# JuliaStats/Klara.jl

Hardware: AMD Instinct MI355X
Metric: MCMC transitions/sec (whole node), 100-dim Gaussian, 65k chains (higher is better)
Workload: dtype f64

## Files before the change

klara.jl_amd/csrc/klara_diagt.h:

```cpp
#pragma once
#include "klara_kernels.h"

#ifndef KLARA_DIAGT_Q
#define KLARA_DIAGT_Q 8
#endif
#define KLARA_DIAGT_CPW (64 / KLARA_DIAGT_Q)
#ifndef KLARA_DT_FENCE_EVERY
#define KLARA_DT_FENCE_EVERY 2
#endif
#ifndef KLARA_DT_SLICE_WF
#define KLARA_DT_SLICE_WF 4
#endif
#ifndef KLARA_DT_W1
#define KLARA_DT_W1 4
#endif
#ifndef KLARA_Q4_MALA_WF
#define KLARA_Q4_MALA_WF 3
#endif
#ifndef KLARA_DT_WF
#define KLARA_DT_WF 2
#endif
#ifdef KLARA_DT_PERSISTENT
#define KLARA_DT_GROUP_LOOP for (long long grp = kl.group0 + wave0; grp < kl.group_end && grp * CPW < p.nchains; grp += nwaves)
#else
#define KLARA_DT_GROUP_LOOP const long long grp = kl.group0 + wave0; if (grp < kl.group_end && grp * CPW < p.nchains)
#endif
#define KLARA_DT_PAIR_FENCE(pi) do { if (KLARA_DT_FENCE_EVERY > 0 && ((pi) + 1) % KLARA_DT_FENCE_EVERY == 0) __builtin_amdgcn_sched_barrier(0); } while (0)

struct KAuto {
    const int* cell_in;
    int* cell_out;
    unsigned long long* acc_ctr;
    int* mirror;
    unsigned long long thr_work;
    int my_mode;
    int fanout;
    int launch_idx;
};
#define KLARA_AUTO_NONE KAuto{ nullptr, nullptr, nullptr, nullptr, 0ull, 0, 1, 0 }

__device__ __forceinline__ unsigned wave_sum_u32(unsigned v)
{
#pragma unroll
    for (int m = 1; m < 64; m <<= 1) v += (unsigned)__builtin_amdgcn_ds_bpermute((int)((((unsigned)threadIdx.x & 63u) ^ (unsigned)m) << 2), (int)v);
    return v;
}
__shared__ unsigned klara_auto_wg[2];
__device__ __forceinline__ void auto_begin()
{
    if (threadIdx.x < 2) klara_auto_wg[threadIdx.x] = 0u;
}
__device__ __forceinline__ void auto_finish(const KAuto& ka, unsigned wave_acc)
{
    if (ka.acc_ctr == nullptr) return;
    const unsigned tot = wave_sum_u32(wave_acc);
    if ((threadIdx.x & 63) == 0) {
        atomicAdd(&klara_auto_wg[0], tot);
        if (atomicAdd(&klara_auto_wg[1], 1u) != (blockDim.x >> 6) - 1) return;
        const unsigned long long wg_tot = atomicAdd(&klara_auto_wg[0], 0u);
        const unsigned long long old = atomicAdd(ka.acc_ctr, (1ull << 40) | wg_tot);
        if ((old >> 40) == (unsigned long long)gridDim.x - 1) {
            const unsigned long long total = (old & ((1ull << 40) - 1)) + wg_tot;
            *ka.acc_ctr = 0ull;
            const int mode = (total << 16) > ka.thr_work ? 1 : 0;
            if (ka.cell_out != nullptr) for (int k = 0; k < ka.fanout; ++k) ka.cell_out[2 * k] = mode;
            if (ka.mirror != nullptr) {
                for (int k = 0; k < ka.fanout; ++k) {
                    __hip_atomic_store(ka.mirror + 4 * k + 1, (int)(total > 0x7fffffffull ? 0x7fffffffull : total), __ATOMIC_RELAXED, __HIP_MEMORY_SCOPE_SYSTEM);
                    __hip_atomic_store(ka.mirror + 4 * k, mode, __ATOMIC_RELAXED, __HIP_MEMORY_SCOPE_SYSTEM);
                    __hip_atomic_store(ka.mirror + 4 * k + 2, ka.launch_idx, __ATOMIC_RELEASE, __HIP_MEMORY_SCOPE_SYSTEM);
                }
            }
        }
    }
}

template <int NP, int Q>
struct PairCtx {
    int lane, q, cw;
    unsigned off0;
    bool last_ok;
    bool last_full;
};

template <int NP, int Q>
__device__ __forceinline__ PairCtx<NP, Q> make_pctx(int D)
{
    PairCtx<NP, Q> c;
    c.lane = threadIdx.x & 63;
    c.q = c.lane & (Q - 1);
    c.cw = c.lane / Q;
    c.off0 = (unsigned)((c.cw * D + 2 * c.q) * 8);
    c.last_ok = 2 * ((NP - 1) * Q + c.q) < D;
    c.last_full = 2 * ((NP - 1) * Q + c.q) + 1 < D;
    return c;
}
template <int NP, int Q>
__device__ __forceinline__ unsigned pair_off(const PairCtx<NP, Q>& c, int p)
{
    const unsigned o = c.off0 + (unsigned)(p * Q * 16);
    return (p == NP - 1 && !c.last_ok) ? KLARA_BUF_OOB : o;
}
template <int NP, int Q>
__device__ __forceinline__ void load_pairs(const PairCtx<NP, Q>& c, __amdgpu_buffer_rsrc_t w, double (&v)[2 * NP])
{
#pragma unroll
    for (int p = 0; p < NP; ++p) {
        const kd_uint4 t = __builtin_amdgcn_raw_buffer_load_b128(w, pair_off<NP, Q>(c, p), 0, 0);
        v[2 * p] = __builtin_bit_cast(double, kd_uint2{ t.x, t.y });
        v[2 * p + 1] = __builtin_bit_cast(double, kd_uint2{ t.z, t.w });
        if (p == NP - 1 && !c.last_full) v[2 * p + 1] = 0.0;
    }
}
template <int NP, int Q>
__device__ __forceinline__ void store_pairs(const PairCtx<NP, Q>& c, __amdgpu_buffer_rsrc_t w, const double (&v)[2 * NP])
{
#pragma unroll
    for (int p = 0; p < NP; ++p) {
        const kd_uint2 a = __builtin_bit_cast(kd_uint2, v[2 * p]), b = __builtin_bit_cast(kd_uint2, v[2 * p + 1]);
        if (p < NP - 1) {
            __builtin_amdgcn_raw_buffer_store_b128(kd_uint4{ a.x, a.y, b.x, b.y }, w, pair_off<NP, Q>(c, p), 0, 0);
        } else {
            const unsigned o = pair_off<NP, Q>(c, p);
            __builtin_amdgcn_raw_buffer_store_b64(a, w, o, 0, 0);
            __builtin_amdgcn_raw_buffer_store_b64(b, w, c.last_full ? o + 8u : KLARA_BUF_OOB, 0, 0);
        }
    }
}
template <int NP, int Q>
__device__ __forceinline__ void load_pairs_if(const PairCtx<NP, Q>& c, __amdgpu_buffer_rsrc_t w, bool on, double (&v)[2 * NP])
{
#pragma unroll
    for (int p = 0; p < NP; ++p) {
        const kd_uint4 t = __builtin_amdgcn_raw_buffer_load_b128(w, on ? pair_off<NP, Q>(c, p) : KLARA_BUF_OOB, 0, 0);
        v[2 * p] = __builtin_bit_cast(double, kd_uint2{ t.x, t.y });
        v[2 * p + 1] = __builtin_bit_cast(double, kd_uint2{ t.z, t.w });
        if (p == NP - 1 && !c.last_full) v[2 * p + 1] = 0.0;
    }
}
template <int NP, int Q>
__device__ __forceinline__ void store_pairs_if(const PairCtx<NP, Q>& c, __amdgpu_buffer_rsrc_t w, bool on, const double (&v)[2 * NP])
{
#pragma unroll
    for (int p = 0; p < NP; ++p) {
        const kd_uint2 a = __builtin_bit_cast(kd_uint2, v[2 * p]), b = __builtin_bit_cast(kd_uint2, v[2 * p + 1]);
        const unsigned o = on ? pair_off<NP, Q>(c, p) : KLARA_BUF_OOB;
        if (p < NP - 1) {
            __builtin_amdgcn_raw_buffer_store_b128(kd_uint4{ a.x, a.y, b.x, b.y }, w, o, 0, 0);
        } else {
            __builtin_amdgcn_raw_buffer_store_b64(a, w, o, 0, 0);
            __builtin_amdgcn_raw_buffer_store_b64(b, w, (on && c.last_full) ? o + 8u : KLARA_BUF_OOB, 0, 0);
        }
    }
}
template <int NP, int Q>
__device__ __forceinline__ void diagt_fold(const PairCtx<NP, Q>& c, __amdgpu_buffer_rsrc_t wsum, __amdgpu_buffer_rsrc_t wsq, bool fold,
                                        bool& loaded, long long& held, const double (&x)[2 * NP], double (&sm)[2 * NP], double (&sq)[2 * NP])
{
    const bool need = fold && !loaded;
    if (__any(need)) {
        double ts[2 * NP], tq[2 * NP];
        load_pairs_if<NP, Q>(c, wsum, need, ts);
        load_pairs_if<NP, Q>(c, wsq, need, tq);
#pragma unroll
        for (int e = 0; e < 2 * NP; ++e) { sm[e] = need ? ts[e] : sm[e]; sq[e] = need ? tq[e] : sq[e]; }
        loaded = loaded || need;
    }
    const double hf = fold ? (double)held : 0.0;
#pragma unroll
    for (int e = 0; e < 2 * NP; ++e) {
        const double a = sm[e] + hf * x[e], b = sq[e] + hf * (x[e] * x[e]);
        sm[e] = fold ? a : sm[e]; sq[e] = fold ? b : sq[e];
    }
    held = fold ? 0 : held;
}

#ifndef KLARA_DT_RMW_CHUNK
#define KLARA_DT_RMW_CHUNK 3
#endif
template <int NP, int Q>
__device__ __forceinline__ void diagt_fold_atomic(const PairCtx<NP, Q>& c, gdouble* sum0, gdouble* sq0, bool fold, long long& held, const double (&x)[2 * NP])
{
    typedef __attribute__((address_space(1))) double* gptr;
    if (fold) {
        const double hf = (double)held;
        const gptr ps = (gptr)((__attribute__((address_space(1))) char*)sum0 + c.off0), pq = (gptr)((__attribute__((address_space(1))) char*)sq0 + c.off0);
#pragma unroll
        for (int p = 0; p < NP; ++p) {
            const bool ok0 = p < NP - 1 || c.last_ok, ok1 = p < NP - 1 || c.last_full;
            if (ok0) {
                (void)__builtin_amdgcn_global_atomic_fadd_f64(ps + p * Q * 2, hf * x[2 * p]);
                (void)__builtin_amdgcn_global_atomic_fadd_f64(pq + p * Q * 2, hf * (x[2 * p] * x[2 * p]));
            }
            if (ok1) {
                (void)__builtin_amdgcn_global_atomic_fadd_f64(ps + p * Q * 2 + 1, hf * x[2 * p + 1]);
                (void)__builtin_amdgcn_global_atomic_fadd_f64(pq + p * Q * 2 + 1, hf * (x[2 * p + 1] * x[2 * p + 1]));
            }
        }
    }
    held = fold ? 0 : held;
}
template <int NP, int Q>
__device__ __forceinline__ void diagt_fold_rmw(const PairCtx<NP, Q>& c, __amdgpu_buffer_rsrc_t wsum, __amdgpu_buffer_rsrc_t wsq, bool fold,
                                               long long& held, const double (&x)[2 * NP])
{
    const double hf = fold ? (double)held : 0.0;
    constexpr int CH = KLARA_DT_RMW_CHUNK;
#pragma unroll
    for (int p0 = 0; p0 < NP; p0 += CH) {
        kd_uint4 ts[CH], tq[CH];
#pragma unroll
        for (int k = 0; k < CH; ++k) {
            if (p0 + k < NP) {
                const unsigned o = fold ? pair_off<NP, Q>(c, p0 + k) : KLARA_BUF_OOB;
                ts[k] = __builtin_amdgcn_raw_buffer_load_b128(wsum, o, 0, 0);
                tq[k] = __builtin_amdgcn_raw_buffer_load_b128(wsq, o, 0, 0);
            }
        }
#pragma unroll
        for (int k = 0; k < CH; ++k) {
            if (p0 + k < NP) {
                const int p = p0 + k;
                const unsigned o = fold ? pair_off<NP, Q>(c, p) : KLARA_BUF_OOB;
                const double s0 = __builtin_bit_cast(double, kd_uint2{ ts[k].x, ts[k].y }) + hf * x[2 * p];
                const double s1 = __builtin_bit_cast(double, kd_uint2{ ts[k].z, ts[k].w }) + hf * x[2 * p + 1];
                const double q0 = __builtin_bit_cast(double, kd_uint2{ tq[k].x, tq[k].y }) + hf * (x[2 * p] * x[2 * p]);
                const double q1 = __builtin_bit_cast(double, kd_uint2{ tq[k].z, tq[k].w }) + hf * (x[2 * p + 1] * x[2 * p + 1]);
                const kd_uint2 a = __builtin_bit_cast(kd_uint2, s0), b = __builtin_bit_cast(kd_uint2, s1);
                const kd_uint2 e = __builtin_bit_cast(kd_uint2, q0), f = __builtin_bit_cast(kd_uint2, q1);
                if (p < NP - 1) {
                    __builtin_amdgcn_raw_buffer_store_b128(kd_uint4{ a.x, a.y, b.x, b.y }, wsum, o, 0, 0);
                    __builtin_amdgcn_raw_buffer_store_b128(kd_uint4{ e.x, e.y, f.x, f.y }, wsq, o, 0, 0);
                } else {
                    const unsigned o1 = (fold && c.last_full) ? o + 8u : KLARA_BUF_OOB;
                    __builtin_amdgcn_raw_buffer_store_b64(a, wsum, o, 0, 0); __builtin_amdgcn_raw_buffer_store_b64(b, wsum, o1, 0, 0);
                    __builtin_amdgcn_raw_buffer_store_b64(e, wsq, o, 0, 0); __builtin_amdgcn_raw_buffer_store_b64(f, wsq, o1, 0, 0);
                }
            }
        }
    }
    held = fold ? 0 : held;
}

template <int NP, int Q>
__device__ __forceinline__ void load_pair_param(const PairCtx<NP, Q>& c, const gdouble* base, int D, double dflt, double (&v)[2 * NP])
{
#pragma unroll
    for (int p = 0; p < NP; ++p) {
        const int i = 2 * (p * Q + c.q);
        v[2 * p] = dflt; v[2 * p + 1] = dflt;
        if (base != nullptr && i < D) v[2 * p] = base[i];
        if (base != nullptr && i + 1 < D) v[2 * p + 1] = base[i + 1];
    }
}

template <int Q> struct PairShare {
    static constexpr int STEP = Q <= 8 ? 8 / Q : 0;
    static constexpr bool second(int p) { return STEP != 0 && ((p / (STEP ? STEP : 1)) & 1) != 0; }
};
template <int NP, int Q>
__device__ __forceinline__ void pair_words(const PairCtx<NP, Q>& c, unsigned long long seed, unsigned long long gchain,
                                           unsigned long long t, int p, uint32_t (&stash)[4], uint32_t& wa, uint32_t& wb)
{
    constexpr int STEP = PairShare<Q>::STEP, S1 = STEP ? STEP : 1;
    if (PairShare<Q>::second(p)) {
        wa = stash[2 * (p % S1)]; wb = stash[2 * (p % S1) + 1];
    } else {
        const uint32_t idx = (uint32_t)(p * Q + c.q);
        const bool pad = p == NP - 1 && !c.last_ok;
        const kd_u32x4 b = kd_stream_block(seed, gchain, t, pad ? idx : kd_pair_block(idx));
        if constexpr (STEP != 0) {
            wa = b.x; wb = b.y;
            stash[2 * (p % S1)] = b.z; stash[2 * (p % S1) + 1] = b.w;
        } else {
            const bool hb = !pad && kd_pair_half(idx) != 0u;
            wa = hb ? b.z : b.x; wb = hb ? b.w : b.y;
        }
    }
}
template <int NP, int Q, bool SCTAB = false>
__device__ __forceinline__ void pair_normals(const PairCtx<NP, Q>& c, unsigned long long seed, unsigned long long gchain,
                                             unsigned long long t, int p, uint32_t (&stash)[4], double& z0, double& z1, double& u1, double& lg1)
{
    uint32_t wa, wb;
    pair_words<NP, Q>(c, seed, gchain, t, p, stash, wa, wb);
    kd_normal_pair_w_t<SCTAB>(wa, wb, &z0, &z1, &u1, &lg1);
    KLARA_PIN(z0); KLARA_PIN(z1);
    if (p == NP - 1 && !c.last_ok) z0 = 0.0;
    if (p == NP - 1 && !c.last_full) z1 = 0.0;
}
template <int NP, int Q>
__device__ __forceinline__ void pair_issue(const PairCtx<NP, Q>& c, unsigned long long seed, unsigned long long gchain,
                                           unsigned long long t, int p, uint32_t (&stash)[4], kd_pair_reads& rd)
{
    uint32_t wa, wb;
    pair_words<NP, Q>(c, seed, gchain, t, p, stash, wa, wb);
    kd_normal_pair_issue(wa, wb, &rd);
    __builtin_amdgcn_sched_barrier(0);
}
template <int NP, int Q>
__device__ __forceinline__ void pair_finish(const PairCtx<NP, Q>& c, int p, const kd_pair_reads& rd, double& z0, double& z1, double& u1, double& lg1)
{
    kd_normal_pair_finish(&rd, &z0, &z1, &u1, &lg1);
    KLARA_PIN(z0); KLARA_PIN(z1);
    if (p == NP - 1 && !c.last_ok) z0 = 0.0;
    if (p == NP - 1 && !c.last_full) z1 = 0.0;
}

template <int V> struct kd_int { static constexpr int value = V; };
template <int FROM, int TO, class F>
__device__ __forceinline__ void kd_static_for(F&& f)
{
    if constexpr (FROM < TO) { f(kd_int<FROM>{}); kd_static_for<FROM + 1, TO>(f); }
}

template <bool UNITW>
__device__ __forceinline__ void diag_elem(double x, double w, double m2w, double m, double& term, double& grad)
{
    const double dd = UNITW ? x : x - m;
    term = UNITW ? dd * dd : w * (dd * dd);
    grad = UNITW ? -2.0 * dd : m2w * dd;
}

template <int SAMPLER, int NP, int Q, bool ONESTEP, bool TUNE>
__host__ __device__ constexpr int diagt_min_waves()
{
    return NP <= 8 ? (ONESTEP && SAMPLER != KLARA_SAMPLER_HMC ? KLARA_DT_W1 : KLARA_DT_WF)
                   : (Q == 4 && NP <= 13 && !TUNE ? (SAMPLER == KLARA_SAMPLER_MALA ? KLARA_Q4_MALA_WF : 2) : 1);
}

#ifndef KLARA_SCTAB_MIN_STEPS
#define KLARA_SCTAB_MIN_STEPS 8
#endif
template <int SAMPLER, int NP, int Q, bool ONESTEP, bool UNITW, bool MON, bool TUNE>
__host__ __device__ constexpr bool diagt_sctab()
{
    return SAMPLER == KLARA_SAMPLER_MALA && ((Q == 4 && NP == 13) || (Q == 8 && NP == 7)) && !ONESTEP && UNITW && MON && !TUNE;
}
#ifndef KLARA_Q4_SCTAB_WG
#define KLARA_Q4_SCTAB_WG 256
#endif
template <int Q, bool SCTAB>
__host__ __device__ constexpr int diagt_wg_threads() { return SCTAB && Q == 4 ? KLARA_Q4_SCTAB_WG : 256; }

#ifdef KLARA_USER_PAIR_TARGET
#define KLARA_PAIR_CALL(a, b, P, g0, g1) klara_user_pair((a), (b), (P), D, (const double*)p.cdata, (long long)p.cndata, (g0), (g1))
#else
#define KLARA_PAIR_CALL(a, b, P, g0, g1) 0.0
#endif
template <int SAMPLER, int NP, int Q, bool ONESTEP, bool UNITW, bool MON, bool TUNE = false, bool DA = false, bool USERPAIR = false, bool SCTAB = false>
__global__ __launch_bounds__((diagt_wg_threads<Q, SCTAB>()), (SAMPLER == KLARA_SAMPLER_SLICE && NP <= 8 && !MON && !TUNE ? KLARA_DT_SLICE_WF : diagt_min_waves<SAMPLER, NP, Q, ONESTEP, TUNE>()))
void k_diagt(const KParams* __restrict__ pp, const KLaunch kl, const KAuto ka)
{
#ifndef KLARA_USER_PAIR_TARGET
    static_assert(!USERPAIR, "pair closures exist in run-time compiled translation units only");
#endif
    static_assert(!USERPAIR || (UNITW && Q >= 8), "pair closures: 8 or more lanes per chain");
    static_assert(!SCTAB || (!ONESTEP && !USERPAIR && SAMPLER != KLARA_SAMPLER_SLICE), "the remainder table: fused launches of the built-in MH / MALA / HMC kernels");
    if (ka.cell_in != nullptr && *ka.cell_in != ka.my_mode) return;
    static_assert(!(ONESTEP && (MON || TUNE)), "monitored / tuned jobs run the committing kernel");
    static_assert(!DA || (TUNE && SAMPLER == KLARA_SAMPLER_HMC), "dual averaging: tuned HMC");
    constexpr bool PLAIN = !TUNE;
    constexpr int E = 2 * NP, CPW = 64 / Q;
    constexpr bool NEEDG = SAMPLER == KLARA_SAMPLER_MALA || SAMPLER == KLARA_SAMPLER_HMC;
    constexpr bool SLICE = SAMPLER == KLARA_SAMPLER_SLICE;
    static_assert(!(SLICE && ONESTEP), "the slice sampler moves every chain: it runs the committing kernel");
    constexpr bool MEMSUM = MON && !TUNE && Q == 4 && (SAMPLER == KLARA_SAMPLER_MH || SAMPLER == KLARA_SAMPLER_MALA);
    const KParams& p = *pp;
    __shared__ __attribute__((aligned(16))) double lds_w[UNITW ? 2 : 2 * NP * Q];
    __shared__ __attribute__((aligned(16))) double lds_mu[UNITW ? 2 : 2 * NP * Q];
    __shared__ __attribute__((aligned(16))) double lds_m2w[UNITW ? 2 : 2 * NP * Q];
    if (!UNITW) {
        for (int i = (int)threadIdx.x; i < 2 * NP * Q; i += (int)blockDim.x) {
            lds_w[i] = (p.gw != nullptr && i < p.D) ? p.gw[i] : 1.0;
            lds_mu[i] = (p.gmu != nullptr && i < p.D) ? p.gmu[i] : 0.0;
            lds_m2w[i] = -2.0 * lds_w[i];
        }
    }
    auto_begin();
    if constexpr (SCTAB) kd_sincos_rem_to_lds();
    kd_tables_to_lds();
    if (p.clock_probe != nullptr && blockIdx.x == (gridDim.x >> 1) && threadIdx.x == 0) {
        p.clock_probe[2] = __builtin_amdgcn_s_memtime(); p.clock_probe[3] = __builtin_amdgcn_s_memrealtime();
    }
    const int D = p.D;
    const PairCtx<NP, Q> cx = make_pctx<NP, Q>(D);
    const int nsteps = ONESTEP ? 1 : kl.nsteps;
    guchar* const accept_out = p.accept != nullptr ? p.accept + kl.t0 * (unsigned long long)p.nchains : nullptr;

    double sig[E];
    const auto wv = [&](int e) { return UNITW ? 1.0 : lds_w[2 * ((e >> 1) * Q + cx.q) + (e & 1)]; };
    const auto mv = [&](int e) { return UNITW ? 0.0 : lds_mu[2 * ((e >> 1) * Q + cx.q) + (e & 1)]; };
    const auto m2wv = [&](int e) { return UNITW ? -2.0 : lds_m2w[2 * ((e >> 1) * Q + cx.q) + (e & 1)]; };
    const auto wvl = [&](int e) { return UNITW ? 1.0 : *(volatile const double*)&lds_w[2 * ((e >> 1) * Q + cx.q) + (e & 1)]; };
    const auto mvl = [&](int e) { return UNITW ? 0.0 : *(volatile const double*)&lds_mu[2 * ((e >> 1) * Q + cx.q) + (e & 1)]; };
    const auto m2wvl = [&](int e) { return UNITW ? -2.0 : *(volatile const double*)&lds_m2w[2 * ((e >> 1) * Q + cx.q) + (e & 1)]; };
    if (SAMPLER == KLARA_SAMPLER_MH) load_pair_param<NP, Q>(cx, p.vecparam, D, 1.0, sig);
    const double gconst = USERPAIR ? 0.0 : p.gconst;

    const int acc_slot = (D + 1) >> 1;
    const bool acc_free = acc_slot < NP * Q && !PairShare<Q>::second(NP - 1);
    const int acc_lane = (cx.lane - cx.q) + (acc_slot & (Q - 1));

    const long long nwaves = (long long)gridDim.x * (blockDim.x >> 6);
    const long long wave0 = __builtin_amdgcn_readfirstlane((int)(blockIdx.x * (blockDim.x >> 6) + (threadIdx.x >> 6)));
    unsigned wave_acc = 0;
    KLARA_DT_GROUP_LOOP {
        const long long first_chain = grp * CPW;
        const long long left = p.nchains - first_chain;
        const int here = left < CPW ? (int)left : CPW;
        const bool chain_ok = cx.cw < here;
        const long long chain = first_chain + cx.cw;
        const unsigned long long gchain = (unsigned long long)(p.chain_offset + chain);
        const __amdgpu_buffer_rsrc_t wx = group_window(p.X, first_chain, here, D);
        const __amdgpu_buffer_rsrc_t wg = group_window(p.GR, first_chain, here, D);

        double x[E];
        load_pairs<NP, Q>(cx, wx, x);
        const auto user_pair = [&](int pi, double a, double b, double& nt, double& g0, double& g1) {
            double u0 = 0.0, u1 = 0.0, u = 0.0;
            const bool ok0 = pi < NP - 1 || cx.last_ok, ok1 = pi < NP - 1 || cx.last_full;
            if (ok0) u = KLARA_PAIR_CALL(a, b, pi * Q + cx.q, &u0, &u1);
            nt = ok0 ? -u : 0.0; g0 = ok0 ? u0 : 0.0; g1 = ok1 ? u1 : 0.0;
        };
        const auto grad_of = [&](const double (&v)[E], double (&out)[E]) {
            if constexpr (USERPAIR) {
#pragma unroll
                for (int pi = 0; pi < NP; ++pi) { double nt; user_pair(pi, v[2 * pi], v[2 * pi + 1], nt, out[2 * pi], out[2 * pi + 1]); }
            } else {
#pragma unroll
                for (int e = 0; e < E; ++e) { double term_; diag_elem<UNITW>(v[e], wv(e), m2wv(e), mv(e), term_, out[e]); }
            }
        };
        double lt = p.LT[chain_ok ? chain : 0];
        unsigned long long nacc = 0;
        bool stuck = false;
        const bool do_sum = MON && p.sum != nullptr;
        double sm[MEMSUM ? 2 : E], sq[MEMSUM ? 2 : E];
        bool sums_loaded = false;
        long long held = 0;
        __amdgpu_buffer_rsrc_t wsum = wx, wsq = wx;
        if (do_sum) {
#pragma unroll
            for (int e = 0; e < (MEMSUM ? 2 : E); ++e) { sm[e] = 0.0; sq[e] = 0.0; }
            wsum = group_window(p.sum, first_chain, here, D); wsq = group_window(p.sumsq, first_chain, here, D);
            held = p.held[chain_ok ? chain : 0];
        }
        int sphase = kl.save_phase0;
        long long scol = kl.save_col0;
        const bool per_chain_tune = KCNT && !KPOOLED;
        const long long c0 = chain_ok ? chain : 0;
        TuneRegs tn;
        if (per_chain_tune) tn = { p.tune_step[c0], p.tune_accepted[c0], p.tune_proposed[c0], p.tune_totproposed[c0], 0, 0.0, 0.0 };
        else if (KPOOLED) tn = { p.tune_step[0], p.tune_accepted[0], 0, 0, 0, 0.0, 0.0 };
        else tn = { DA ? p.tune_step[c0] : p.step0, 0, 0, 0, 0, 0.0, 0.0 };
        if (DA) { tn.epsbar = p.da_epsbar[c0]; tn.hbar = p.da_hbar[c0]; }
        const long long acc0 = tn.accepted;
        tn.phase = per_chain_tune ? (int)(tn.proposed % p.period) : 0;

        struct { unsigned long long seed; long long burnin, nsteps_total, hist_cols, held_inc; int thinning; double sqrt_step0, inv_step0; } lc = {};
        if constexpr (SCTAB) {
            lc.seed = p.seed; lc.burnin = p.burnin; lc.nsteps_total = p.nsteps_total; lc.hist_cols = p.hist_cols; lc.thinning = (int)p.thinning;
            lc.held_inc = __builtin_amdgcn_readfirstlane(do_sum ? 1 : 0); lc.sqrt_step0 = p.sqrt_step0; lc.inv_step0 = p.inv_step0;
            KLARA_PIN_S(lc.seed); KLARA_PIN_S(lc.burnin); KLARA_PIN_S(lc.nsteps_total); KLARA_PIN_S(lc.hist_cols); KLARA_PIN_S(lc.thinning);
            KLARA_PIN_S(lc.held_inc); KLARA_PIN_S(lc.sqrt_step0); KLARA_PIN_S(lc.inv_step0);
        }
#define KLARA_LC(f) (SCTAB ? lc.f : p.f)
        for (int s = 0; s < nsteps; ++s) {
            const unsigned long long t = kl.t0 + (unsigned long long)s;
            if (KCNT) tune_count_proposal(p, tn);
            double xp[E];
            const auto put_xp = [&](int pi, double a, double b) { xp[2 * pi] = a; xp[2 * pi + 1] = b; };
            constexpr int NR = Q == 4 ? 2 : 1;
            double red[3 * NR] = {}, red1[1], red2[2];
            double u_last = 0.5, lg_last = 0.0;
            uint32_t nstash[4] = { 0u, 0u, 0u, 0u };
            bool acc;
            double ltp, a_da = 0.0;

            constexpr bool ZFIRST = (ONESTEP || Q != 4) && SAMPLER != KLARA_SAMPLER_HMC && !SLICE;
            double z[ZFIRST ? E : 2];
            kd_pair_reads rd[2];
            if (ZFIRST) {
                if constexpr (SCTAB) pair_issue<NP, Q>(cx, KLARA_LC(seed), gchain, t, 0, nstash, rd[0]);
#pragma unroll
                for (int pi = 0; pi < NP; ++pi) {
                    if constexpr (SCTAB) {
                        if (pi + 1 < NP) pair_issue<NP, Q>(cx, KLARA_LC(seed), gchain, t, pi + 1, nstash, rd[(pi + 1) & 1]);
                        pair_finish<NP, Q>(cx, pi, rd[pi & 1], z[2 * pi], z[2 * pi + 1], u_last, lg_last);
                        __builtin_amdgcn_sched_barrier(0);
                    } else {
                        pair_normals<NP, Q, SCTAB>(cx, KLARA_LC(seed), gchain, t, pi, nstash, z[2 * pi], z[2 * pi + 1], u_last, lg_last);
                        KLARA_DT_PAIR_FENCE(pi);
                    }
                }
            }
            if constexpr (SLICE) {
                if (do_sum && __any(held > 0))
                    diagt_fold<NP, Q>(cx, wsum, wsq, held > 0, sums_loaded, held, x, sm, sq);
            }
            if (SLICE) {
                acc = true;
                const __amdgpu_buffer_rsrc_t wwid = __builtin_amdgcn_make_buffer_rsrc((void*)p.vecparam, 0, D * 8, 0x00020000);
#pragma unroll
                for (int e = 0; e < E; ++e) {
                    const int i = 2 * ((e >> 1) * Q + cx.q) + (e & 1);
                    const bool live = chain_ok && i < D;
                    const uint32_t base = (uint32_t)(live ? i : 0) << KLARA_SLICE_ATT_BITS;
                    const kd_u32x4 b0 = kd_stream_block(KLARA_LC(seed), gchain, t, base);
                    const double lgu = kd_log_u01(kd_uniform_xy(b0));
                    const double ru = kd_uniform_zw(b0);
                    const double wi_t = UNITW ? 1.0 : wv(e), mi_t = UNITW ? 0.0 : mv(e);
                    const double xi = x[e], wd = __builtin_bit_cast(double, __builtin_amdgcn_raw_buffer_load_b64(wwid, (unsigned)(live ? i : 0) * 8u, 0, 0));
                    double tcur, gd_;
                    if constexpr (USERPAIR) { double g1_; user_pair(e >> 1, x[e & ~1], x[e | 1], tcur, gd_, g1_); }
                    else diag_elem<UNITW>(xi, wi_t, -2.0 * wi_t, mi_t, tcur, gd_);
                    double Li = xi - ru * wd;
                    double Ri = xi + (1.0 - ru) * wd;
                    const auto term_of = [&](double cand) -> double {
                        double tc, gd;
                        if constexpr (USERPAIR) { double g1; user_pair(e >> 1, (e & 1) ? x[e & ~1] : cand, (e & 1) ? cand : x[e | 1], tc, gd, g1); }
                        else diag_elem<UNITW>(cand, wi_t, -2.0 * wi_t, mi_t, tc, gd);
                        return tc;
                    };
                    if (p.stepout) {
                        double dl = tcur - term_of(Li);
                        int guard = 0;
                        while (true) {
                            bool go = live && !stuck && (dl > lgu);
                            if (go && ++guard > KLARA_SLICE_MAX_ATT) { stuck = true; go = false; }
                            if (!__any(go)) break;
                            const double Ln = Li - wd;
                            const double dn = tcur - term_of(go ? Ln : Li);
                            if (go) { Li = Ln; dl = dn; }
                        }
                        double dr = tcur - term_of(Ri);
                        guard = 0;
                        while (true) {
                            bool go = live && !stuck && (dr > lgu);
                            if (go && ++guard > KLARA_SLICE_MAX_ATT) { stuck = true; go = false; }
                            if (!__any(go)) break;
                            const double Rn = Ri + wd;
                            const double dn = tcur - term_of(go ? Rn : Ri);
                            if (go) { Ri = Rn; dr = dn; }
                        }
                    }
                    double xprime = xi;
                    bool done = !live || stuck;
                    kd_u32x4 ab = b0;
                    for (uint32_t a = 1;; ++a) {
                        if (!done && a > KLARA_SLICE_MAX_ATT) { stuck = true; done = true; }
                        if (!__any(!done)) break;
                        if (a & 1u) ab = kd_stream_block(KLARA_LC(seed), gchain, t, kd_slice_attempt_slot(base, a));
                        const double u = (a & 1u) ? kd_uniform_xy(ab) : kd_uniform_zw(ab);
                        const double cand = u * (Ri - Li) + Li;
                        const double tc = term_of(done ? xprime : cand);
                        if (!done) {
                            xprime = cand;
                            if (tcur - tc > lgu) done = true;
                            else if (cand > xi) Ri = cand;
                            else if (cand < xi) Li = cand;
                            else { stuck = true; done = true; }
                        }
                    }
                    if (live && !stuck) x[e] = xprime;
                }
                red1[0] = 0.0;
                if constexpr (USERPAIR) {
#pragma unroll
                    for (int pi = 0; pi < NP; ++pi) { double nt, g0_, g1_; user_pair(pi, x[2 * pi], x[2 * pi + 1], nt, g0_, g1_); red1[0] = red1[0] + nt; }
                } else {
#pragma unroll
                for (int e = 0; e < E; ++e) { double te, gd; diag_elem<UNITW>(x[e], wv(e), m2wv(e), mv(e), te, gd); red1[0] = red1[0] + te; }
                }
                group_allreduce<1>(red1, Q, cx.lane);
                lt = gconst - red1[0];
                ltp = lt;
#pragma unroll
                for (int e = 0; e < E; ++e) xp[e] = x[e];
            } else if (SAMPLER == KLARA_SAMPLER_MH) {
                const auto mh_elem = [&](int e, double ze, int r) -> double {
                    const double xe = x[e] + sig[e] * ze;
                    double term, gd;
                    diag_elem<UNITW>(xe, wv(e), m2wv(e), mv(e), term, gd);
                    red[r] = red[r] + term;
                    return xe;
                };
#pragma unroll
                for (int pi = 0; pi < NP; ++pi) {
                    double z0 = ZFIRST ? z[(2 * pi) % (ZFIRST ? E : 2)] : 0.0, z1 = ZFIRST ? z[(2 * pi + 1) % (ZFIRST ? E : 2)] : 0.0;
                    if (!ZFIRST) pair_normals<NP, Q, SCTAB>(cx, KLARA_LC(seed), gchain, t, pi, nstash, z0, z1, u_last, lg_last);
                    const int r = (NR == 2 && (pi & 1)) ? 3 : 0;
                    if constexpr (USERPAIR) {
                        const double a = x[2 * pi] + sig[2 * pi] * z0, b = x[2 * pi + 1] + sig[2 * pi + 1] * z1;
                        double nt, g0, g1;
                        user_pair(pi, a, b, nt, g0, g1);
                        red[r] = red[r] + nt;
                        put_xp(pi, a, b);
                    } else {
                        const double a = mh_elem(2 * pi, z0, r), b = mh_elem(2 * pi + 1, z1, r);
                        put_xp(pi, a, b);
                    }
                    if (!ZFIRST) KLARA_DT_PAIR_FENCE(pi);
                }
                if (NR == 2) {
                    red2[0] = red[0]; red2[1] = red[3];
                    group_allreduce<2>(red2, Q, cx.lane);
                    red1[0] = red2[0] + red2[1];
                } else {
                    red1[0] = red[0];
                    group_allreduce<1>(red1, Q, cx.lane);
                }
                ltp = gconst - red1[0];
                const double ratio = ltp - lt;
                acc = ratio > 0.0;
                if (acc_free) acc = acc || ratio > lane_bcast(lg_last, acc_lane);
                else if (!acc && ratio > KD_LOG_UMIN_GUARD)
                    acc = ratio > kd_log_u01(kd_accept_uniform(kd_stream_block(KLARA_LC(seed), gchain, t, (uint32_t)acc_slot)));
            } else if (SAMPLER == KLARA_SAMPLER_MALA) {
                const double h_ = tn.step, halfh = 0.5 * h_, sq = KCNT ? __builtin_sqrt(h_) : KLARA_LC(sqrt_step0);
                const double half_inv_h = 0.5 * (KCNT ? 1.0 / h_ : KLARA_LC(inv_step0));
                const double neg_h = -h_;
                constexpr bool FROM_TERM = UNITW && PLAIN;
                const auto mala_elem = [&](int e, double ze, int r, bool first) -> double {
                    double term, ge = 0.0, gpe;
                    if constexpr (!UNITW) diag_elem<UNITW>(x[e], wv(e), m2wv(e), mv(e), term, ge);
                    const double m_ = UNITW ? x[e] + neg_h * x[e] : x[e] + halfh * ge;
                    const double xe = m_ + sq * ze;
                    diag_elem<UNITW>(xe, wv(e), m2wv(e), mv(e), term, gpe);
                    red[r] = first ? term : red[r] + term;
                    const double q1 = m_ - xe;
                    red[r + 1] = first ? (q1 * q1) * half_inv_h : red[r + 1] + (q1 * q1) * half_inv_h;
                    const double mup = UNITW ? xe + neg_h * xe : xe + halfh * gpe;
                    const double q2 = mup - x[e];
                    red[r + 2] = first ? (q2 * q2) * half_inv_h : red[r + 2] + (q2 * q2) * half_inv_h;
                    return xe;
                };
#pragma unroll
                for (int pi = 0; pi < NP; ++pi) {
                    double z0 = ZFIRST ? z[(2 * pi) % (ZFIRST ? E : 2)] : 0.0, z1 = ZFIRST ? z[(2 * pi + 1) % (ZFIRST ? E : 2)] : 0.0;
                    if constexpr (!ZFIRST && SCTAB) {
                        if (pi == 0) pair_issue<NP, Q>(cx, KLARA_LC(seed), gchain, t, 0, nstash, rd[0]);
                        pair_finish<NP, Q>(cx, pi, rd[pi & 1], z0, z1, u_last, lg_last);
                        if (pi + 1 < NP) pair_issue<NP, Q>(cx, KLARA_LC(seed), gchain, t, pi + 1, nstash, rd[(pi + 1) & 1]);
                    } else if (!ZFIRST) pair_normals<NP, Q, SCTAB>(cx, KLARA_LC(seed), gchain, t, pi, nstash, z0, z1, u_last, lg_last);
                    const int r = (NR == 2 && (pi & 1)) ? 3 : 0;
                    if constexpr (USERPAIR) {
                        double nt, ge0, ge1, gp0, gp1;
                        user_pair(pi, x[2 * pi], x[2 * pi + 1], nt, ge0, ge1);
                        const double m0 = x[2 * pi] + halfh * ge0, m1 = x[2 * pi + 1] + halfh * ge1;
                        const double a = m0 + sq * z0, b = m1 + sq * z1;
                        user_pair(pi, a, b, nt, gp0, gp1);
                        red[r] = red[r] + nt;
                        const double q10 = m0 - a, q11 = m1 - b;
                        red[r + 1] = red[r + 1] + (q10 * q10) * half_inv_h;
                        red[r + 1] = red[r + 1] + (q11 * q11) * half_inv_h;
                        const double q20 = (a + halfh * gp0) - x[2 * pi], q21 = (b + halfh * gp1) - x[2 * pi + 1];
                        red[r + 2] = red[r + 2] + (q20 * q20) * half_inv_h;
                        red[r + 2] = red[r + 2] + (q21 * q21) * half_inv_h;
                        put_xp(pi, a, b);
                    } else {
                        const double a = mala_elem(2 * pi, z0, r, FROM_TERM && pi < NR), b = mala_elem(2 * pi + 1, z1, r, false);
                        put_xp(pi, a, b);
                    }
                    if constexpr (!ZFIRST && SCTAB) __builtin_amdgcn_sched_barrier(0);
                    else if (!ZFIRST) KLARA_DT_PAIR_FENCE(pi);
                }
                group_allreduce<3 * NR>(red, Q, cx.lane);
                if (NR == 2) { red[0] = red[0] + red[3]; red[1] = red[1] + red[4]; red[2] = red[2] + red[5]; }
                ltp = gconst - red[0];
                double ratio = ltp - lt;
                ratio += red[1];
                ratio -= red[2];
                acc = ratio > 0.0;
                if (acc_free) acc = acc || ratio > lane_bcast(lg_last, acc_lane);
                else if (!acc && ratio > KD_LOG_UMIN_GUARD)
                    acc = ratio > kd_log_u01(kd_accept_uniform(kd_stream_block(KLARA_LC(seed), gchain, t, (uint32_t)acc_slot)));
            } else {
                const double eps = tn.step, halfe = 0.5 * eps;
                double mom[E], gp[E];
                double k0[NR] = {};
#pragma unroll
                for (int pi = 0; pi < NP; ++pi) {
                    pair_normals<NP, Q, SCTAB>(cx, KLARA_LC(seed), gchain, t, pi, nstash, mom[2 * pi], mom[2 * pi + 1], u_last, lg_last);
                    const int r = (NR == 2 && (pi & 1)) ? 1 : 0;
                    k0[r] = k0[r] + mom[2 * pi] * mom[2 * pi];
                    k0[r] = k0[r] + mom[2 * pi + 1] * mom[2 * pi + 1];
                }
                group_allreduce<NR>(k0, Q, cx.lane);
                if (NR == 2) k0[0] = k0[0] + k0[1];
                const double H0 = lt - 0.5 * k0[0];
#pragma unroll
                for (int e = 0; e < E; ++e) xp[e] = x[e];
                constexpr bool KFOLD = UNITW && !USERPAIR;
                if constexpr (!KFOLD) grad_of(x, gp);
                const int nl = DA ? (chain_ok ? da_nleaps(p, eps) : 1) : p.nleaps;
#pragma unroll
                for (int e = 0; e < E; ++e) {
                    if constexpr (KFOLD) mom[e] = kd_fma(-eps, x[e], mom[e]);
                    else mom[e] = kd_fma(halfe, gp[e], mom[e]);
                }
                const int nlmax = DA ? wave_max_int(nl) : nl;
                for (int l = 0; l < nlmax; ++l) {
                    const bool go = !DA || l < nl;
                    const double kf = l + 1 < nl ? eps : halfe;
                    const double nkf2 = -2.0 * kf;
                    if constexpr (USERPAIR) {
#pragma unroll
                        for (int pi = 0; pi < NP; ++pi) {
                            const double xa = kd_fma(eps, mom[2 * pi], xp[2 * pi]), xb = kd_fma(eps, mom[2 * pi + 1], xp[2 * pi + 1]);
                            xp[2 * pi] = go ? xa : xp[2 * pi]; xp[2 * pi + 1] = go ? xb : xp[2 * pi + 1];
                            double nt, ga, gb;
                            user_pair(pi, xp[2 * pi], xp[2 * pi + 1], nt, ga, gb);
                            gp[2 * pi] = go ? ga : gp[2 * pi]; gp[2 * pi + 1] = go ? gb : gp[2 * pi + 1];
                            const double na = kd_fma(kf, gp[2 * pi], mom[2 * pi]), nb = kd_fma(kf, gp[2 * pi + 1], mom[2 * pi + 1]);
                            mom[2 * pi] = go ? na : mom[2 * pi]; mom[2 * pi + 1] = go ? nb : mom[2 * pi + 1];
                        }
                    } else {
#pragma unroll
                        for (int e = 0; e < E; ++e) {
                            const double x1 = kd_fma(eps, mom[e], xp[e]);
                            xp[e] = go ? x1 : xp[e];
                            if constexpr (KFOLD) {
                                const double m2 = kd_fma(nkf2, xp[e], mom[e]);
                                mom[e] = go ? m2 : mom[e];
                            } else {
                                double term, g1;
                                diag_elem<UNITW>(xp[e], 1.0, m2wvl(e), mvl(e), term, g1);
                                gp[e] = go ? g1 : gp[e];
                                const double m2 = kd_fma(kf, gp[e], mom[e]);
                                mom[e] = go ? m2 : mom[e];
                            }
                        }
                    }
                }
                if constexpr (USERPAIR) {
#pragma unroll
                    for (int pi = 0; pi < NP; ++pi) {
                        double nt, ga, gb;
                        user_pair(pi, xp[2 * pi], xp[2 * pi + 1], nt, ga, gb);
                        red[0] = red[0] + nt;
                        red[1] = red[1] + mom[2 * pi] * mom[2 * pi];
                        red[1] = red[1] + mom[2 * pi + 1] * mom[2 * pi + 1];
                    }
                } else {
#pragma unroll
                for (int e = 0; e < E; ++e) {
                    double term, gd;
                    diag_elem<UNITW>(xp[e], wv(e), m2wv(e), mv(e), term, gd);
                    const int r = (NR == 2 && ((e >> 1) & 1)) ? 3 : 0;
                    red[r] = red[r] + term;
                    red[r + 1] = red[r + 1] + mom[e] * mom[e];
                }
                }
                if (NR == 2) {
                    double red4[4] = { red[0], red[1], red[3], red[4] };
                    group_allreduce<4>(red4, Q, cx.lane);
                    red2[0] = red4[0] + red4[2]; red2[1] = red4[1] + red4[3];
                } else {
                    red2[0] = red[0]; red2[1] = red[1];
                    group_allreduce<2>(red2, Q, cx.lane);
                }
                ltp = gconst - red2[0];
                const double H1 = ltp - 0.5 * red2[1];
                const double ratio = H1 - H0;
                const double ex = kd_exp(ratio);
                const double a = 1.0 < ex ? 1.0 : ex;
                a_da = a;
                const double u = acc_free ? lane_bcast(u_last, acc_lane)
                                          : kd_accept_uniform(kd_stream_block(KLARA_LC(seed), gchain, t, (uint32_t)acc_slot));
                acc = u < a;
            }

            if (accept_out != nullptr && chain_ok && cx.q == 0) accept_out[(long long)s * p.nchains + chain] = acc ? 1 : 0;
            if (KCNT && acc && !SLICE) tn.accepted += 1;
            if (DA) da_update(p, tn, (long long)t + 1, a_da);
            if (per_chain_tune && !DA) tuning_block(p, tn);
            else if (DA && per_chain_tune && tn.phase == 0 && (long long)t + 1 <= p.da_nadapt) {
                tn.totproposed += tn.proposed; tn.accepted = 0; tn.proposed = 0;
            }
            if constexpr (ONESTEP) {
                wave_acc += (acc && chain_ok && cx.q == 0) ? 1u : 0u;
                if (acc) {
                    store_pairs<NP, Q>(cx, wx, xp);
                    if (NEEDG) { double gq[E]; grad_of(xp, gq); store_pairs<NP, Q>(cx, wg, gq); }
                    if (chain_ok && cx.q == 0) { p.LT[chain] = ltp; p.naccept[chain] += 1ull; }
                }
            } else {
                nacc += acc ? 1ull : 0ull;
                if (!SLICE && do_sum && __any(chain_ok && acc && held > 0)) {
                    const bool fold = chain_ok && acc && held > 0;
#ifdef KLARA_DT_FOLD_RMW
                    if constexpr (MEMSUM) diagt_fold_rmw<NP, Q>(cx, wsum, wsq, fold, held, x);
#else
                    if constexpr (MEMSUM) diagt_fold_atomic<NP, Q>(cx, p.sum + first_chain * D, p.sumsq + first_chain * D, fold, held, x);
#endif
                    else diagt_fold<NP, Q>(cx, wsum, wsq, fold, sums_loaded, held, x, sm, sq);
                }
                if (acc) {
#pragma unroll
                    for (int e = 0; e < E; ++e) x[e] = xp[e];
                    lt = ltp;
                }
            }
            const long long i1 = (long long)t + 1;
            if (MON && i1 > KLARA_LC(burnin) && i1 <= KLARA_LC(nsteps_total)) {
                if (sphase == 0) {
                    if constexpr (SCTAB) held += lc.held_inc;
                    else if (do_sum) held += 1;
                    if (scol < KLARA_LC(hist_cols)) {
                        const long long col0 = scol * p.nchains + first_chain;
                        if (p.hist != nullptr) store_pairs<NP, Q>(cx, group_window(p.hist, col0, here, D), x);
                        if (NEEDG && p.hist_g != nullptr) { double gq[E]; grad_of(x, gq); store_pairs<NP, Q>(cx, group_window(p.hist_g, col0, here, D), gq); }
                        if (p.hist_lt != nullptr && chain_ok && cx.q == 0) p.hist_lt[scol * p.nchains + chain] = lt;
                    }
                    ++scol;
                }
                sphase = (sphase + 1 == (SCTAB ? lc.thinning : (int)p.thinning)) ? 0 : sphase + 1;
            }
        }
        if (do_sum) {
            if constexpr (!MEMSUM) {
                if (__any(sums_loaded)) {
                    store_pairs_if<NP, Q>(cx, wsum, sums_loaded, sm);
                    store_pairs_if<NP, Q>(cx, wsq, sums_loaded, sq);
                }
            }
            if (chain_ok && cx.q == 0) p.held[chain] = held;
        }
        if (SLICE && stuck && chain_ok) klara_raise(p.error_flag, KLARA_ERR_SLICE_STUCK);
        if (!ONESTEP) wave_acc += (chain_ok && cx.q == 0) ? (unsigned)nacc : 0u;
        if (!ONESTEP && nacc != 0) {
            store_pairs<NP, Q>(cx, wx, x);
            if (NEEDG) { double gq[E]; grad_of(x, gq); store_pairs<NP, Q>(cx, wg, gq); }
            if (chain_ok && cx.q == 0) { p.LT[chain] = lt; p.naccept[chain] += nacc; }
        }
        if (TUNE && chain_ok && cx.q == 0) {
            if (DA) { p.tune_step[chain] = tn.step; p.da_epsbar[chain] = tn.epsbar; p.da_hbar[chain] = tn.hbar; }
            if (per_chain_tune) {
                p.tune_step[chain] = tn.step; p.tune_accepted[chain] = tn.accepted;
                p.tune_proposed[chain] = tn.proposed; p.tune_totproposed[chain] = tn.totproposed;
            } else if (KPOOLED && KCNT) {
                atomicAdd((unsigned long long*)p.pooled_accepted, (unsigned long long)(tn.accepted - acc0));
            }
        }
    }
    if (p.clock_probe != nullptr && blockIdx.x == (gridDim.x >> 1) && threadIdx.x == 0) {
        p.clock_probe[0] = __builtin_amdgcn_s_memtime(); p.clock_probe[1] = __builtin_amdgcn_s_memrealtime();
    }
    auto_finish(ka, wave_acc);
#undef KLARA_LC
}

template <int NP, int Q, bool USERPAIR = false>
__global__ __launch_bounds__(256) void k_diagt_init(const KParams p, int needgrad)
{
#ifndef KLARA_USER_PAIR_TARGET
    static_assert(!USERPAIR, "pair closures exist in run-time compiled translation units only");
#endif
    constexpr int E = 2 * NP, CPW = 64 / Q;
    const int D = p.D;
    const PairCtx<NP, Q> cx = make_pctx<NP, Q>(D);
    const long long grp = __builtin_amdgcn_readfirstlane((int)(blockIdx.x * (blockDim.x >> 6) + (threadIdx.x >> 6)));
    const long long first_chain = grp * CPW;
    const long long left = p.nchains - first_chain;
    const int here = left < CPW ? (left > 0 ? (int)left : 0) : CPW;
    const bool chain_ok = cx.cw < here;
    const long long chain = first_chain + cx.cw;
    double w[E], mu[E], x[E], g[E], red[1] = { 0.0 };
    load_pair_param<NP, Q>(cx, p.gw, D, 1.0, w);
    load_pair_param<NP, Q>(cx, p.gmu, D, 0.0, mu);
    load_pairs<NP, Q>(cx, group_window(p.X, first_chain, here, D), x);
    bool bad = false;
    if constexpr (USERPAIR) {
#pragma unroll
        for (int pi = 0; pi < NP; ++pi) {
            double u0 = 0.0, u1 = 0.0, u = 0.0;
            const bool ok0 = pi < NP - 1 || cx.last_ok, ok1 = pi < NP - 1 || cx.last_full;
            if (ok0) u = KLARA_PAIR_CALL(x[2 * pi], x[2 * pi + 1], pi * Q + cx.q, &u0, &u1);
            red[0] = red[0] + (ok0 ? -u : 0.0);
            g[2 * pi] = ok0 ? u0 : 0.0; g[2 * pi + 1] = ok1 ? u1 : 0.0;
            bad = bad || !kfinite(g[2 * pi]) || !kfinite(g[2 * pi + 1]);
        }
    } else {
#pragma unroll
    for (int e = 0; e < E; ++e) {
        double term;
        diag_elem<false>(x[e], w[e], -2.0 * w[e], mu[e], term, g[e]);
        red[0] = red[0] + term;
        bad = bad || !kfinite(g[e]);
    }
    }
    group_allreduce<1>(red, Q, cx.lane);
    const double lt = (USERPAIR ? 0.0 : p.gconst) - red[0];
    bad = chain_ok && ((needgrad && bad) || !kfinite(lt));
    if (needgrad) store_pairs<NP, Q>(cx, group_window(p.GR, first_chain, here, D), g);
    if (chain_ok && cx.q == 0) p.LT[chain] = lt;
    if (bad) klara_raise(p.error_flag, KLARA_ERR_NONFINITE_INIT);
}
```

Before: 6.084 billion.

## Cut register pressure in the fused MALA remainder-table kernel

For the fused SCTAB MALA kernel, the lane context used at the end of the step loop and for history and accept stores is now recomputed late from mbcnt instead of being held live across the loop. Scalar loop constants (half inverse step, acc_free, and save window bounds precomputed as step indices) are pinned in SGPRs. An optional cache of kept drift means is added but disabled by default, and a separate min-waves knob is introduced for the Q4 SCTAB variant. The aim is to free VGPRs so more waves can be resident. The cost is some recomputation of lane indices and extra code paths to maintain.

Measured after the change: 6.164 billion, median of 6. 1.01x the previous value.

```diff
diff --git a/klara.jl_amd/csrc/klara_diagt.h b/klara.jl_amd/csrc/klara_diagt.h
--- a/klara.jl_amd/csrc/klara_diagt.h
+++ b/klara.jl_amd/csrc/klara_diagt.h
@@ -16,6 +16,9 @@
 #endif
 #ifndef KLARA_Q4_MALA_WF
 #define KLARA_Q4_MALA_WF 3
+#endif
+#ifndef KLARA_Q4_SCTAB_WF
+#define KLARA_Q4_SCTAB_WF 3
 #endif
 #ifndef KLARA_DT_WF
 #define KLARA_DT_WF 2
@@ -96,6 +99,18 @@
     return c;
 }
 template <int NP, int Q>
+__device__ __forceinline__ PairCtx<NP, Q> make_pctx_at(int D, int lane)
+{
+    PairCtx<NP, Q> c;
+    c.lane = lane;
+    c.q = c.lane & (Q - 1);
+    c.cw = c.lane / Q;
+    c.off0 = (unsigned)((c.cw * D + 2 * c.q) * 8);
+    c.last_ok = 2 * ((NP - 1) * Q + c.q) < D;
+    c.last_full = 2 * ((NP - 1) * Q + c.q) + 1 < D;
+    return c;
+}
+template <int NP, int Q>
 __device__ __forceinline__ unsigned pair_off(const PairCtx<NP, Q>& c, int p)
 {
     const unsigned o = c.off0 + (unsigned)(p * Q * 16);
@@ -322,10 +337,11 @@
     grad = UNITW ? -2.0 * dd : m2w * dd;
 }
 
-template <int SAMPLER, int NP, int Q, bool ONESTEP, bool TUNE>
+template <int SAMPLER, int NP, int Q, bool ONESTEP, bool TUNE, bool SCTAB = false>
 __host__ __device__ constexpr int diagt_min_waves()
 {
-    return NP <= 8 ? (ONESTEP && SAMPLER != KLARA_SAMPLER_HMC ? KLARA_DT_W1 : KLARA_DT_WF)
+    return SCTAB && Q == 4 && NP > 8 ? KLARA_Q4_SCTAB_WF
+         : NP <= 8 ? (ONESTEP && SAMPLER != KLARA_SAMPLER_HMC ? KLARA_DT_W1 : KLARA_DT_WF)
                    : (Q == 4 && NP <= 13 && !TUNE ? (SAMPLER == KLARA_SAMPLER_MALA ? KLARA_Q4_MALA_WF : 2) : 1);
 }
 
@@ -342,6 +358,17 @@
 #endif
 template <int Q, bool SCTAB>
 __host__ __device__ constexpr int diagt_wg_threads() { return SCTAB && Q == 4 ? KLARA_Q4_SCTAB_WG : 256; }
+#ifndef KLARA_Q4_KEPT_MEANS
+#define KLARA_Q4_KEPT_MEANS 0
+#endif
+#ifndef KLARA_Q8_KEPT_MEANS
+#define KLARA_Q8_KEPT_MEANS 0
+#endif
+template <int SAMPLER, int NP, int Q, bool UNITW, bool TUNE, bool SCTAB>
+__host__ __device__ constexpr int diagt_kept_means()
+{
+    return SCTAB && SAMPLER == KLARA_SAMPLER_MALA && UNITW && !TUNE ? (Q == 4 ? KLARA_Q4_KEPT_MEANS : Q == 8 ? KLARA_Q8_KEPT_MEANS : 0) : 0;
+}
 
 #ifdef KLARA_USER_PAIR_TARGET
 #define KLARA_PAIR_CALL(a, b, P, g0, g1) klara_user_pair((a), (b), (P), D, (const double*)p.cdata, (long long)p.cndata, (g0), (g1))
@@ -349,7 +376,7 @@
 #define KLARA_PAIR_CALL(a, b, P, g0, g1) 0.0
 #endif
 template <int SAMPLER, int NP, int Q, bool ONESTEP, bool UNITW, bool MON, bool TUNE = false, bool DA = false, bool USERPAIR = false, bool SCTAB = false>
-__global__ __launch_bounds__((diagt_wg_threads<Q, SCTAB>()), (SAMPLER == KLARA_SAMPLER_SLICE && NP <= 8 && !MON && !TUNE ? KLARA_DT_SLICE_WF : diagt_min_waves<SAMPLER, NP, Q, ONESTEP, TUNE>()))
+__global__ __launch_bounds__((diagt_wg_threads<Q, SCTAB>()), (SAMPLER == KLARA_SAMPLER_SLICE && NP <= 8 && !MON && !TUNE ? KLARA_DT_SLICE_WF : diagt_min_waves<SAMPLER, NP, Q, ONESTEP, TUNE, SCTAB>()))
 void k_diagt(const KParams* __restrict__ pp, const KLaunch kl, const KAuto ka)
 {
 #ifndef KLARA_USER_PAIR_TARGET
@@ -364,6 +391,8 @@
     constexpr int E = 2 * NP, CPW = 64 / Q;
     constexpr bool NEEDG = SAMPLER == KLARA_SAMPLER_MALA || SAMPLER == KLARA_SAMPLER_HMC;
     constexpr bool SLICE = SAMPLER == KLARA_SAMPLER_SLICE;
+    constexpr int KM = diagt_kept_means<SAMPLER, NP, Q, UNITW, TUNE, SCTAB>();
+    static_assert(KM >= 0 && KM <= E, "kept drift means: a prefix of the lane's elements");
     static_assert(!(SLICE && ONESTEP), "the slice sampler moves every chain: it runs the committing kernel");
     constexpr bool MEMSUM = MON && !TUNE && Q == 4 && (SAMPLER == KLARA_SAMPLER_MH || SAMPLER == KLARA_SAMPLER_MALA);
     const KParams& p = *pp;
@@ -417,6 +446,13 @@
 
         double x[E];
         load_pairs<NP, Q>(cx, wx, x);
+        const auto late_ctx = [&]() -> PairCtx<NP, Q> {
+            if constexpr (SCTAB && Q == 4) {
+                int l = (int)__builtin_amdgcn_mbcnt_hi(~0u, __builtin_amdgcn_mbcnt_lo(~0u, 0u));
+                KLARA_PIN(l);
+                return make_pctx_at<NP, Q>(D, l & 63);
+            } else return cx;
+        };
         const auto user_pair = [&](int pi, double a, double b, double& nt, double& g0, double& g1) {
             double u0 = 0.0, u1 = 0.0, u = 0.0;
             const bool ok0 = pi < NP - 1 || cx.last_ok, ok1 = pi < NP - 1 || cx.last_full;
@@ -458,14 +494,28 @@
         const long long acc0 = tn.accepted;
         tn.phase = per_chain_tune ? (int)(tn.proposed % p.period) : 0;
 
-        struct { unsigned long long seed; long long burnin, nsteps_total, hist_cols, held_inc; int thinning; double sqrt_step0, inv_step0; } lc = {};
+        struct { unsigned long long seed; long long hist_cols, held_inc; int thinning, acc_free, save_lo, save_hi; double sqrt_step0, half_inv_step0; } lc = {};
         if constexpr (SCTAB) {
-            lc.seed = p.seed; lc.burnin = p.burnin; lc.nsteps_total = p.nsteps_total; lc.hist_cols = p.hist_cols; lc.thinning = (int)p.thinning;
-            lc.held_inc = __builtin_amdgcn_readfirstlane(do_sum ? 1 : 0); lc.sqrt_step0 = p.sqrt_step0; lc.inv_step0 = p.inv_step0;
-            KLARA_PIN_S(lc.seed); KLARA_PIN_S(lc.burnin); KLARA_PIN_S(lc.nsteps_total); KLARA_PIN_S(lc.hist_cols); KLARA_PIN_S(lc.thinning);
-            KLARA_PIN_S(lc.held_inc); KLARA_PIN_S(lc.sqrt_step0); KLARA_PIN_S(lc.inv_step0);
+            lc.seed = p.seed; lc.hist_cols = p.hist_cols; lc.thinning = (int)p.thinning;
+            lc.held_inc = __builtin_amdgcn_readfirstlane(do_sum ? 1 : 0); lc.sqrt_step0 = p.sqrt_step0;
+            KLARA_PIN_S(lc.seed); KLARA_PIN_S(lc.hist_cols); KLARA_PIN_S(lc.thinning);
+            KLARA_PIN_S(lc.held_inc); KLARA_PIN_S(lc.sqrt_step0);
+            const kd_uint2 hih = __builtin_bit_cast(kd_uint2, 0.5 * p.inv_step0);
+            lc.half_inv_step0 = __builtin_bit_cast(double, kd_uint2{ (uint32_t)__builtin_amdgcn_readfirstlane((int)hih.x), (uint32_t)__builtin_amdgcn_readfirstlane((int)hih.y) });
+            KLARA_PIN_S(lc.half_inv_step0);
+            lc.acc_free = __builtin_amdgcn_readfirstlane(acc_free ? 1 : 0);
+            KLARA_PIN_S(lc.acc_free);
+            const long long lo = (long long)p.burnin - (long long)kl.t0, hi = (long long)p.nsteps_total - (long long)kl.t0;
+            lc.save_lo = (int)(lo < 0 ? 0 : lo > nsteps ? nsteps : lo); lc.save_hi = (int)(hi < 0 ? 0 : hi > nsteps ? nsteps : hi);
+            KLARA_PIN_S(lc.save_lo); KLARA_PIN_S(lc.save_hi);
         }
 #define KLARA_LC(f) (SCTAB ? lc.f : p.f)
+        double dm[KM > 0 ? KM : 1];
+        const double neg_h_kept = KM > 0 ? -tn.step : 0.0;
+        if constexpr (KM > 0) {
+#pragma unroll
+            for (int e = 0; e < KM; ++e) dm[e] = x[e] + neg_h_kept * x[e];
+        }
         for (int s = 0; s < nsteps; ++s) {
             const unsigned long long t = kl.t0 + (unsigned long long)s;
             if (KCNT) tune_count_proposal(p, tn);
@@ -619,13 +669,13 @@
                     acc = ratio > kd_log_u01(kd_accept_uniform(kd_stream_block(KLARA_LC(seed), gchain, t, (uint32_t)acc_slot)));
             } else if (SAMPLER == KLARA_SAMPLER_MALA) {
                 const double h_ = tn.step, halfh = 0.5 * h_, sq = KCNT ? __builtin_sqrt(h_) : KLARA_LC(sqrt_step0);
-                const double half_inv_h = 0.5 * (KCNT ? 1.0 / h_ : KLARA_LC(inv_step0));
+                const double half_inv_h = SCTAB ? lc.half_inv_step0 : 0.5 * (KCNT ? 1.0 / h_ : p.inv_step0);
                 const double neg_h = -h_;
                 constexpr bool FROM_TERM = UNITW && PLAIN;
                 const auto mala_elem = [&](int e, double ze, int r, bool first) -> double {
                     double term, ge = 0.0, gpe;
                     if constexpr (!UNITW) diag_elem<UNITW>(x[e], wv(e), m2wv(e), mv(e), term, ge);
-                    const double m_ = UNITW ? x[e] + neg_h * x[e] : x[e] + halfh * ge;
+                    const double m_ = UNITW ? (e < KM ? dm[e < KM ? e : 0] : x[e] + neg_h * x[e]) : x[e] + halfh * ge;
                     const double xe = m_ + sq * ze;
                     diag_elem<UNITW>(xe, wv(e), m2wv(e), mv(e), term, gpe);
                     red[r] = first ? term : red[r] + term;
@@ -673,9 +723,13 @@
                 ratio += red[1];
                 ratio -= red[2];
                 acc = ratio > 0.0;
-                if (acc_free) acc = acc || ratio > lane_bcast(lg_last, acc_lane);
-                else if (!acc && ratio > KD_LOG_UMIN_GUARD)
-                    acc = ratio > kd_log_u01(kd_accept_uniform(kd_stream_block(KLARA_LC(seed), gchain, t, (uint32_t)acc_slot)));
+                if (SCTAB ? lc.acc_free != 0 : acc_free) acc = acc || ratio > lane_bcast(lg_last, acc_lane);
+                else {
+                    double guard = KD_LOG_UMIN_GUARD;
+                    if constexpr (SCTAB) KLARA_PIN_S(guard);
+                    if (!acc && ratio > guard)
+                        acc = ratio > kd_log_u01(kd_accept_uniform(kd_stream_block(KLARA_LC(seed), gchain, t, (uint32_t)acc_slot)));
+                }
             } else {
                 const double eps = tn.step, halfe = 0.5 * eps;
                 double mom[E], gp[E];
@@ -772,7 +826,12 @@
                 acc = u < a;
             }
 
-            if (accept_out != nullptr && chain_ok && cx.q == 0) accept_out[(long long)s * p.nchains + chain] = acc ? 1 : 0;
+            if constexpr (SCTAB) {
+                if (accept_out != nullptr) {
+                    const PairCtx<NP, Q> cxa = late_ctx();
+                    if (cxa.cw < here && cxa.q == 0) accept_out[(long long)s * p.nchains + (first_chain + cxa.cw)] = acc ? 1 : 0;
+                }
+            } else if (accept_out != nullptr && chain_ok && cx.q == 0) accept_out[(long long)s * p.nchains + chain] = acc ? 1 : 0;
             if (KCNT && acc && !SLICE) tn.accepted += 1;
             if (DA) da_update(p, tn, (long long)t + 1, a_da);
             if (per_chain_tune && !DA) tuning_block(p, tn);
@@ -800,40 +859,50 @@
                 if (acc) {
 #pragma unroll
                     for (int e = 0; e < E; ++e) x[e] = xp[e];
+                    if constexpr (KM > 0) {
+#pragma unroll
+                        for (int e = 0; e < KM; ++e) dm[e] = xp[e] + neg_h_kept * xp[e];
+                    }
                     lt = ltp;
                 }
             }
             const long long i1 = (long long)t + 1;
-            if (MON && i1 > KLARA_LC(burnin) && i1 <= KLARA_LC(nsteps_total)) {
+            if (MON && (SCTAB ? s >= lc.save_lo && s < lc.save_hi : i1 > p.burnin && i1 <= p.nsteps_total)) {
                 if (sphase == 0) {
                     if constexpr (SCTAB) held += lc.held_inc;
                     else if (do_sum) held += 1;
                     if (scol < KLARA_LC(hist_cols)) {
                         const long long col0 = scol * p.nchains + first_chain;
-                        if (p.hist != nullptr) store_pairs<NP, Q>(cx, group_window(p.hist, col0, here, D), x);
-                        if (NEEDG && p.hist_g != nullptr) { double gq[E]; grad_of(x, gq); store_pairs<NP, Q>(cx, group_window(p.hist_g, col0, here, D), gq); }
-                        if (p.hist_lt != nullptr && chain_ok && cx.q == 0) p.hist_lt[scol * p.nchains + chain] = lt;
+                        const PairCtx<NP, Q> cxh = late_ctx();
+                        if (p.hist != nullptr) store_pairs<NP, Q>(cxh, group_window(p.hist, col0, here, D), x);
+                        if (NEEDG && p.hist_g != nullptr) { double gq[E]; grad_of(x, gq); store_pairs<NP, Q>(cxh, group_window(p.hist_g, col0, here, D), gq); }
+                        if constexpr (SCTAB) {
+                            if (p.hist_lt != nullptr && cxh.cw < here && cxh.q == 0) p.hist_lt[scol * p.nchains + (first_chain + cxh.cw)] = lt;
+                        } else if (p.hist_lt != nullptr && chain_ok && cx.q == 0) p.hist_lt[scol * p.nchains + chain] = lt;
                     }
                     ++scol;
                 }
                 sphase = (sphase + 1 == (SCTAB ? lc.thinning : (int)p.thinning)) ? 0 : sphase + 1;
             }
         }
+        const PairCtx<NP, Q> cxe = late_ctx();
+        const bool chain_ok_e = SCTAB ? cxe.cw < here : chain_ok;
+        const long long chain_e = SCTAB ? first_chain + cxe.cw : chain;
         if (do_sum) {
             if constexpr (!MEMSUM) {
                 if (__any(sums_loaded)) {
-                    store_pairs_if<NP, Q>(cx, wsum, sums_loaded, sm);
-                    store_pairs_if<NP, Q>(cx, wsq, sums_loaded, sq);
-                }
-            }
-            if (chain_ok && cx.q == 0) p.held[chain] = held;
+                    store_pairs_if<NP, Q>(cxe, wsum, sums_loaded, sm);
+                    store_pairs_if<NP, Q>(cxe, wsq, sums_loaded, sq);
+                }
+            }
+            if (chain_ok_e && cxe.q == 0) p.held[chain_e] = held;
         }
         if (SLICE && stuck && chain_ok) klara_raise(p.error_flag, KLARA_ERR_SLICE_STUCK);
-        if (!ONESTEP) wave_acc += (chain_ok && cx.q == 0) ? (unsigned)nacc : 0u;
+        if (!ONESTEP) wave_acc += (chain_ok_e && cxe.q == 0) ? (unsigned)nacc : 0u;
         if (!ONESTEP && nacc != 0) {
-            store_pairs<NP, Q>(cx, wx, x);
-            if (NEEDG) { double gq[E]; grad_of(x, gq); store_pairs<NP, Q>(cx, wg, gq); }
-            if (chain_ok && cx.q == 0) { p.LT[chain] = lt; p.naccept[chain] += nacc; }
+            store_pairs<NP, Q>(cxe, wx, x);
+            if (NEEDG) { double gq[E]; grad_of(x, gq); store_pairs<NP, Q>(cxe, wg, gq); }
+            if (chain_ok_e && cxe.q == 0) { p.LT[chain_e] = lt; p.naccept[chain_e] += nacc; }
         }
         if (TUNE && chain_ok && cx.q == 0) {
             if (DA) { p.tune_step[chain] = tn.step; p.da_epsbar[chain] = tn.epsbar; p.da_hbar[chain] = tn.hbar; }
```
